# JJKK1313/DiTreeOnlinePlanner

Measured on AMD Instinct MI355X. Metric: candidate tree-expansions/sec (carmaze, H=32), higher is better.
Workload: dtype f16x3; 1 GPU; cfgs/carmaze.yaml + fm_policy flow sampler (K=1), batch=1024 candidates per GPU, H=32 (4 chunks x 8 steps), boxes.csv 20x20, 1024-node tree snapshot, seeded random weights; batch_per_gpu=1024, global_batch=1024, edge_length=32, action_horizon=8, pred_horizon=64, flow_steps=1, tree_nodes=1024, parallelism=candidates sharded x1

## Files before the change

### ditreeonlineplanner_amd/csrc/conv_tiles.hip

```cpp
#include <type_traits>

#include "denoise_device.h"

static thread_local bool g_dn_dry_run = false;
void denoise_set_dry_run(bool on) { g_dn_dry_run = on; }
bool denoise_dry_run() { return g_dn_dry_run; }

template <int PREC>
__device__ __forceinline__ void gemm_epilogue(const ConvGemmParams& p, f32x16_t (&acc)[2][4], char* smem, int tm, int tn,
                                              int tid, int lane, int r5, int h, int wm, int wn,
                                              long long out_extra_bytes = 0) {

  constexpr int ET = PREC == 2 ? 1 : 0;
  float satm = 0.0f;
  const int c_l = wn * 128 + 4 * r5;
  const int n0 = tn * 256 + c_l;
  const bool n_ok = n0 < p.N;
  float bias4[4] = {0.f, 0.f, 0.f, 0.f};
  if (p.bias != nullptr && n_ok) {
    f32x4_t t = *(const f32x4_t*)(p.bias + n0);
#pragma unroll
    for (int j = 0; j < 4; ++j) bias4[j] = t[j];
  }
#pragma unroll
// ... 352 lines not shown
#pragma unroll
      for (int i = 0; i < 16; ++i) acc[mb][j][i] = 0.0f;

  const int swl = (r5 >> 1) & 7;
  const int a_row_off = (wm * 64 + r5) * 128;
  const int b_row_off = 32768 + (wn * 128 + r5) * 128;

  auto kstep = [&](const char* sb, auto stage_tag, char* snext) {
    constexpr bool STAGE = decltype(stage_tag)::value;
    if constexpr (PREC != 1) {
      short8_t af[2][2], bfr[2][4];
      auto rd = [&](int ks, int slot) {
        const int ps = (((ks << 1) | h) ^ swl) << 4;
#pragma unroll
        for (int mb = 0; mb < 2; ++mb)
          af[slot][mb] = *(const short8_t*)(sb + a_row_off + mb * 4096 + ps);
#pragma unroll
        for (int j = 0; j < 4; ++j)
          bfr[slot][j] = *(const short8_t*)(sb + b_row_off + j * 4096 + ps);
      };
      if constexpr (STAGE) {
#pragma unroll
        for (int q = 0; q < 8; ++q) stage_piece(q, snext);
      }
      rd(0, 0);
#pragma unroll
      for (int ks = 0; ks < 4; ++ks) {
        if (ks < 3) rd(ks + 1, (ks + 1) & 1);
#pragma unroll
        for (int mb = 0; mb < 2; ++mb)
#pragma unroll
          for (int j = 0; j < 4; ++j)
            acc[mb][j] = mfma32<ET>(af[ks & 1][mb], bfr[ks & 1][j], acc[mb][j]);
      }
      if constexpr (STAGE) __builtin_amdgcn_sched_group_barrier(0x020, 8, 0);
      __builtin_amdgcn_sched_group_barrier(0x100, 6, 0);
#pragma unroll
      for (int ks = 0; ks < 4; ++ks) {
        if (ks < 3) __builtin_amdgcn_sched_group_barrier(0x100, 6, 0);
        __builtin_amdgcn_sched_group_barrier(0x008, 8, 0);
      }
    } else {
#pragma unroll
      for (int sl = 0; sl < 8; ++sl) {
        const int ps = (sl ^ swl) << 4;
        f32x4_t af[2], bfr[4];
#pragma unroll
        for (int mb = 0; mb < 2; ++mb) af[mb] = *(const f32x4_t*)(sb + a_row_off + mb * 4096 + ps);
#pragma unroll
        for (int j = 0; j < 4; ++j) bfr[j] = *(const f32x4_t*)(sb + b_row_off + j * 4096 + ps);
#pragma unroll
        for (int s2 = 0; s2 < 2; ++s2) {
#pragma unroll
          for (int mb = 0; mb < 2; ++mb) {
            const float a = h ? af[mb][2 * s2 + 1] : af[mb][2 * s2];
#pragma unroll
            for (int j = 0; j < 4; ++j) {
              const float bv = h ? bfr[j][2 * s2 + 1] : bfr[j][2 * s2];
              acc[mb][j] = __builtin_amdgcn_mfma_f32_32x32x2f32(a, bv, acc[mb][j], 0, 0, 0);
            }
          }
        }
        if constexpr (STAGE) stage_piece(sl, snext);
      }
    }
  };

#pragma unroll
  for (int q = 0; q < 8; ++q) stage_piece(q, smem);
  advance();
  for (int kt = 0; kt < nk - 1; ++kt) {
    asm volatile("s_waitcnt vmcnt(0)" ::: "memory");
    __syncthreads();
    kstep(smem + (kt & 1) * 65536, std::true_type{}, smem + ((kt + 1) & 1) * 65536);
    advance();
  }
  asm volatile("s_waitcnt vmcnt(0)" ::: "memory");
  __syncthreads();
  kstep(smem + ((nk - 1) & 1) * 65536, std::false_type{}, nullptr);
  __syncthreads();
  gemm_epilogue<PREC>(p, acc, smem, tm, tn, tid, lane, r5, h, wm, wn, out_extra);
}

template <int ET, bool SPLIT, bool SHORT = false>
__device__ __forceinline__ void gemm_epilogue16(const ConvGemmParams& p, f32x4_t (&acc)[4][8], char* smem, int tm, int tn,
                                                int tid, int lane, int r4, int h4, int wm, int wn) {
  const int c_l = wn * 128 + 8 * r4;
  const int n0 = tn * 256 + c_l;
  {
    f32x4_t b0 = {0.f, 0.f, 0.f, 0.f}, b1 = b0;
    if (p.bias != nullptr) { b0 = *(const f32x4_t*)(p.bias + n0); b1 = *(const f32x4_t*)(p.bias + n0 + 4); }
    if constexpr (ET == 1) {
      const float ws = p.w_scale;
#pragma unroll
      for (int mb = 0; mb < 4; ++mb)
#pragma unroll
        for (int j = 0; j < 4; ++j) { acc[mb][j] = acc[mb][j] * ws + b0[j]; acc[mb][4 + j] = acc[mb][4 + j] * ws + b1[j]; }
    } else if (p.bias != nullptr) {
#pragma unroll
      for (int mb = 0; mb < 4; ++mb)
#pragma unroll
        for (int j = 0; j < 4; ++j) { acc[mb][j] += b0[j]; acc[mb][4 + j] += b1[j]; }
    }
  }
  constexpr bool short_l = SHORT;
  const int lane_b = short_l ? (4 * h4) / p.L : 0, lane_l = -lane_b * p.L;
  int blk_b[4], blk_l[4];
#pragma unroll
  for (int mb = 0; mb < 4; ++mb) {
    const int m0 = tm * 256 + wm * 64 + mb * 16;
    const int b = m0 / p.L;
    blk_b[mb] = b;
    blk_l[mb] = m0 - b * p.L;
  }
  auto store_row = [&](char* o, const float (&v)[8]) {
    short8_t hi, lo;
    if constexpr (ET == 1) {
      sat_check_row(p.sat, v);
#pragma unroll
      for (int jj = 0; jj < 4; ++jj) {
        const f32x2_t c = {__builtin_amdgcn_fmed3f(v[2 * jj], -65504.0f, 65504.0f),
                           __builtin_amdgcn_fmed3f(v[2 * jj + 1], -65504.0f, 65504.0f)};
        const half2_t h = __builtin_convertvector(c, half2_t);
        const short2_t hs = __builtin_bit_cast(short2_t, h);
        hi[2 * jj] = hs[0]; hi[2 * jj + 1] = hs[1];
        if constexpr (SPLIT) {
          const half2_t l = __builtin_convertvector(c - __builtin_convertvector(h, f32x2_t), half2_t);
          const short2_t ls = __builtin_bit_cast(short2_t, l);
          lo[2 * jj] = ls[0]; lo[2 * jj + 1] = ls[1];
        }
      }
    } else {
#pragma unroll
      for (int j = 0; j < 8; ++j) {
        hi[j] = (short)f2bf(v[j]);
        if constexpr (SPLIT) lo[j] = (short)f2bf(v[j] - bf2f((unsigned short)hi[j]));
      }
    }
    *(short8_t*)o = hi;
    if constexpr (SPLIT) *(short8_t*)(o + p.out_plane) = lo;
  };
  auto out_ptr = [&](int mb, int esize) {
    const long long orow = (long long)(blk_b[mb] + lane_b) * p.out_Lp + (long long)(blk_l[mb] + 4 * h4 + lane_l) * p.out_stride + p.out_off;
    return (char*)p.Out + (orow * p.ldc + p.out_coff + n0) * esize;
  };
  if (p.mode < MODE_GN_MISH) {
    const int esize = p.out_f32 ? 4 : 2;
    const long long ostep = (long long)p.out_stride * p.ldc * esize;
#pragma unroll
    for (int mb = 0; mb < 4; ++mb) {
      char* ob = out_ptr(mb, esize);
#pragma unroll
      for (int i = 0; i < 4; ++i, ob += ostep) {
        float v[8];
#pragma unroll
        for (int j = 0; j < 8; ++j) v[j] = acc[mb][j][i];
        if (p.out_f32) {
          *(f32x4_t*)ob = f32x4_t{v[0], v[1], v[2], v[3]};
          *(f32x4_t*)(ob + 16) = f32x4_t{v[4], v[5], v[6], v[7]};
        } else {
          store_row(ob, v);
        }
      }
    }
    return;
  }
  const bool has_film = p.mode == MODE_GN_MISH_FILM, has_res = p.mode == MODE_GN_MISH_RES;
  const int spt = 256 / p.L;
  const int ns = spt > 16 ? spt * 4 : 64;
  float* s_sum = (float*)smem;
  float* s_sq = s_sum + ns;
  float* s_gb = s_sq + ns;
  float* s_film = s_gb + 512;
  const bool film_direct = has_film && short_l;
  const int b_last = p.M / p.L - 1;
  for (int i = tid; i < 2 * ns; i += 512) s_sum[i] = 0.0f;
  s_gb[tid] = tid < 256 ? p.gamma[tn * 256 + tid] : p.beta[tn * 256 + tid - 256];
  if (has_film && !film_direct) {
    for (int idx = tid; idx < spt * 128; idx += 512) {
      const int sm = idx >> 7, c4 = idx & 127;
      const int b = min(tm * spt + sm, b_last);
      const float* src = p.film + (long long)b * p.film_ld + p.film_off + tn * 256 + (c4 & 63) * 4 + (c4 >> 6) * p.N;
      *(f32x4_t*)(s_film + sm * 512 + c4 * 4) = *(const f32x4_t*)src;
    }
  }
  f32x4_t rh[2], rl[2];
  const long long rstep = (long long)p.ldres * 2;
  auto fetch_film = [&](int mb) {
    const float* fr = p.film + (long long)min(blk_b[mb] + lane_b, b_last) * p.film_ld + p.film_off + n0;
    rh[0] = *(const f32x4_t*)fr; rh[1] = *(const f32x4_t*)(fr + 4);
    rl[0] = *(const f32x4_t*)(fr + p.N); rl[1] = *(const f32x4_t*)(fr + p.N + 4);
  };
  if (film_direct) fetch_film(0);
  auto fetch_res = [&](int r) {
    const long long rrow = (long long)(blk_b[r >> 2] + lane_b) * p.res_Lp + blk_l[r >> 2] + 4 * h4 + lane_l + p.res_off;
    const char* rp = (const char*)p.Res + (rrow * p.ldres + n0) * 2 + (r & 3) * rstep;
    rh[r & 1] = *(const f32x4_t*)rp;
    if constexpr (SPLIT) rl[r & 1] = *(const f32x4_t*)(rp + p.res_plane);
  };
  if (has_res) { fetch_res(0); fetch_res(1); }
  __syncthreads();
  const int gi = c_l / p.group_ch;
  const bool wide = p.group_ch >= 128;
  const float inv_cnt = 1.0f / (float)(p.group_ch * p.L);
  int slot[4];
#pragma unroll
  for (int mb = 0; mb < 4; ++mb) slot[mb] = (blk_b[mb] + lane_b - tm * spt) * 4 + gi;
  const bool ordered = !short_l && (p.L >= 128 || (p.group_ch == 256 && p.L >= 32));
  const int hsame = short_l ? (p.L == 8 ? 2 : 1) : 4;
  const bool adder = (r4 == 0 || (!wide && r4 == 8)) && (h4 & (hsame - 1)) == 0;
  const int ocell = ((wm * 2 + wn) * 4 + gi) * 2;
  auto block_sums = [&](float (&s)[4], float* cell) {
#pragma unroll
    for (int mb = 0; mb < 4; ++mb) s[mb] = dpp_add<0xB1>(s[mb]);
#pragma unroll
    for (int mb = 0; mb < 4; ++mb) s[mb] = dpp_add<0x4E>(s[mb]);
#pragma unroll
    for (int mb = 0; mb < 4; ++mb) s[mb] = dpp_add<0x141>(s[mb]);
    if (wide) {
#pragma unroll
      for (int mb = 0; mb < 4; ++mb) s[mb] = dpp_add<0x140>(s[mb]);
    }
    if (hsame >= 2) {
#pragma unroll
      for (int mb = 0; mb < 4; ++mb) s[mb] += __shfl_xor(s[mb], 16);
    }
    if (hsame == 4) {
#pragma unroll
      for (int mb = 0; mb < 4; ++mb) s[mb] += __shfl_xor(s[mb], 32);
    }
    if (ordered) {
      if (p.L >= 64) { s[0] = (s[0] + s[1]) + (s[2] + s[3]); s[2] = 0.0f; }
      else { s[0] += s[1]; s[2] += s[3]; }
      if (adder) { cell[ocell] = s[0]; cell[ocell + 1] = s[2]; }
    } else if (adder) {
#pragma unroll
      for (int mb = 0; mb < 4; ++mb) atomicAdd(&cell[slot[mb]], s[mb]);
    }
  };
  auto cell_sums = [&](const float* cell, float (&t)[4]) {
    if (!ordered) {
#pragma unroll
      for (int mb = 0; mb < 4; ++mb) t[mb] = cell[slot[mb]];
      return;
    }
#pragma unroll
    for (int mb = 0; mb < 4; mb += 2) {
      const int r0 = (blk_b[mb] - tm * spt) * p.L;
      const int w0 = r0 >> 6, nw = p.L >= 64 ? p.L >> 6 : 1, sub = (r0 >> 5) & 1;
      float v = 0.0f;
      for (int w = w0; w < w0 + nw; ++w) {
        v += cell[((w * 2 + 0) * 4 + gi) * 2 + sub];
        v += cell[((w * 2 + 1) * 4 + gi) * 2 + sub];
      }
      t[mb] = v; t[mb + 1] = v;
    }
  };
  float mean_[4], rstd_[4];
  auto pair = [&](int mb, int j, int ip) { return f32x2_t{acc[mb][j][2 * ip], acc[mb][j][2 * ip + 1]}; };
  if constexpr (!SPLIT) {
    float s[4], q[4];
#pragma unroll
    for (int mb = 0; mb < 4; ++mb) {
      f32x2_t s2 = {0.f, 0.f}, q2 = {0.f, 0.f};
#pragma unroll
      for (int j = 0; j < 8; ++j)
#pragma unroll
        for (int ip = 0; ip < 2; ++ip) {
          const f32x2_t v = pair(mb, j, ip);
          s2 += v;
          q2 = __builtin_elementwise_fma(v, v, q2);
        }
      s[mb] = s2[0] + s2[1];
      q[mb] = q2[0] + q2[1];
    }
    block_sums(s, s_sum);
    block_sums(q, s_sq);
    __syncthreads();
    cell_sums(s_sum, s);
    cell_sums(s_sq, q);
#pragma unroll
    for (int mb = 0; mb < 4; ++mb) {
      mean_[mb] = s[mb] * inv_cnt;
      const float var = fmaxf(q[mb] * inv_cnt - mean_[mb] * mean_[mb], 0.0f);
// ... 108 lines not shown
template <int ET>
__device__ __forceinline__ void mm16_snake(f32x4_t (&acc)[4][8], const short8_t (&a)[4], const short8_t (&b)[4], int half) {
#pragma unroll
  for (int mb = 0; mb < 4; ++mb)
#pragma unroll
    for (int jj = 0; jj < 4; ++jj) {
      const int j = (mb & 1) ? 3 - jj : jj;
      acc[mb][half * 4 + j] = mfma16<ET>(a[mb], b[j], acc[mb][half * 4 + j]);
    }
}

#ifdef HALO16_STAMP
__device__ unsigned long long g_halo_stamp[8];
extern "C" int ditree_debug_halo_stamp(unsigned long long* out) {
  return (int)hipMemcpyFromSymbol(out, HIP_SYMBOL(g_halo_stamp), sizeof(g_halo_stamp));
}
__device__ unsigned int g_x3_phase[8][32];
extern "C" int ditree_debug_x3_phase(unsigned int* out) {
  return (int)hipMemcpyFromSymbol(out, HIP_SYMBOL(g_x3_phase), sizeof(g_x3_phase));
}
#define X3_STAMP_MAX 65536
__device__ unsigned long long g_x3_stamp[X3_STAMP_MAX][6];
__device__ unsigned int g_x3_count;
extern "C" int ditree_debug_x3_stamp(unsigned long long* out, unsigned int* count, int reset) {
  int rc = (int)hipMemcpyFromSymbol(count, HIP_SYMBOL(g_x3_count), 4);
  if (rc == 0 && out != nullptr) rc = (int)hipMemcpyFromSymbol(out, HIP_SYMBOL(g_x3_stamp), sizeof(unsigned long long) * 6 * X3_STAMP_MAX);
  if (rc == 0 && reset) { unsigned int z = 0; rc = (int)hipMemcpyToSymbol(HIP_SYMBOL(g_x3_count), &z, 4); }
  return rc;
}
#endif
template <int ET>
__global__ void __launch_bounds__(512, 2) conv3_halo16_kernel(ConvGemmParams p) {
  extern __shared__ __attribute__((aligned(16))) char smem[];
  constexpr int A_BUF = 40960, W_BUF = 32768, W_BASE = 2 * A_BUF;
  const int tid = threadIdx.x, lane = tid & 63;
  const int w = __builtin_amdgcn_readfirstlane(tid >> 6);
  const int r4 = lane & 15, h4 = lane >> 4;
  const int wm = w >> 1, wn = w & 1;
  const int ntn = (p.N + 255) >> 8;
  const int ntm = (p.M + 255) >> 8;
  const int tile = xcd_remap_strips(blockIdx.x, ntm, ntn, p.xcd_strips);
  const int tm = tile / ntn, tn = tile - tm * ntn;
  const int L = p.L, Lp = p.in_Lp, S = 256 / L;
  const int a_rows = S * Lp;
  const int nc = p.Cin >> 6;
  const long long K = 3LL * p.Cin;

  unsigned pa0, pa4, pb;
  const char* const a_base = (const char*)p.A + ((long long)tm * S * Lp + p.in_off) * p.lda * 2;
  const char* const w_base = (const char*)p.W + ((long long)tn * 256) * K * 2;
  const __amdgpu_buffer_rsrc_t a_rsrc = __builtin_amdgcn_make_buffer_rsrc((void*)a_base, 0, 0x7fffffff, 0x00020000);
  const __amdgpu_buffer_rsrc_t w_rsrc = __builtin_amdgcn_make_buffer_rsrc((void*)w_base, 0, 0x7fffffff, 0x00020000);
  {
    const int r = w * 8 + (lane >> 3);
    const int slot = (lane & 7) ^ (r & 7);
    pa0 = (unsigned)((r * p.lda + slot * 8) * 2);
    const int r4r = r + 256;
    const int rs = r4r < a_rows ? r4r : a_rows - 1;
    pa4 = (unsigned)((rs * p.lda + slot * 8) * 2);
  }
  const int a_piece = 64 * p.lda * 2;
  long long wq[4];
  {
    const int lr = lane >> 3;
    const int slot = (lane & 7) ^ lr;
    pb = (unsigned)(((long long)(8 * lr) * K + slot * 8) * 2);
#pragma unroll
    for (int q = 0; q < 4; ++q) {
      const int r0 = (w * 4 + q) * 8;
      const int cu = (r0 & 128) + 8 * (r0 & 8) + ((r0 >> 4) & 7);
      wq[q] = (long long)cu * K * 2;
    }
  }
  const int w_tap = p.Cin * 2;
  auto issue_a = [&](int c, int i) {
    __builtin_amdgcn_raw_ptr_buffer_load_lds(a_rsrc, (LDS_AS void*)(smem + (c & 1) * A_BUF + (w + 8 * i) * 1024), 16,
                                             i < 4 ? pa0 : pa4, c * 128 + (i < 4 ? i * a_piece : 0), 0, 0);
  };
  auto issue_w = [&](int c, int t, int q) {
    __builtin_amdgcn_raw_ptr_buffer_load_lds(w_rsrc, (LDS_AS void*)(smem + W_BASE + ((c + t) & 1) * W_BUF + (w * 4 + q) * 1024),
                                             16, pb, (int)wq[q] + c * 128 + t * w_tap, 0, 0);
  };

  int lrow0;
  {
    const int ml = wm * 64 + r4;
    const int sb = ml / L;
    lrow0 = sb * Lp + (ml - sb * L);
  }
  int lstep[4];
#pragma unroll
  for (int mb = 0; mb < 4; ++mb) lstep[mb] = 16 * mb + 2 * (((wm * 64 + 16 * mb) / L) - ((wm * 64) / L));
  const int swl = r4 & 7;
  const int b_row_off = (wn * 128 + r4) * 128;

  f32x4_t acc[4][8];
#pragma unroll
  for (int mb = 0; mb < 4; ++mb)
#pragma unroll
    for (int j = 0; j < 8; ++j) acc[mb][j] = f32x4_t{0.f, 0.f, 0.f, 0.f};

  short8_t af[2][4], bq[2][4];
  auto rdA = [&](int set, int c, int t, int ks) {
    const char* ab = smem + (c & 1) * A_BUF;
#pragma unroll
    for (int mb = 0; mb < 4; ++mb) {
      const int row = lrow0 + lstep[mb] + t;
      const int ps = (((ks << 2) | h4) ^ (row & 7)) << 4;
      af[set][mb] = *(const short8_t*)(ab + row * 128 + ps);
    }
  };
  auto rdB = [&](int set, int c, int t, int ks, int half) {
    const char* wb = smem + W_BASE + ((c + t) & 1) * W_BUF + b_row_off + half * 8192;
    const int psb = (((ks << 2) | h4) ^ swl) << 4;
#pragma unroll
    for (int jj = 0; jj < 4; ++jj) bq[set][jj] = *(const short8_t*)(wb + jj * 2048 + psb);
  };
  auto mm = [&](int aset, int bset, int half, int mb, int jj) {
    acc[mb][half * 4 + jj] = mfma16<ET>(af[aset][mb], bq[bset][jj], acc[mb][half * 4 + jj]);
  };
  auto mm16 = [&](int aset, int bset, int half) { mm16_snake<ET>(acc, af[aset], bq[bset], half); };

  auto step = [&](auto tT, auto tNext, auto tIW, auto tIA, auto tVM, int c) {
    constexpr int T = decltype(tT)::value;
    constexpr bool HAS_NEXT = decltype(tNext)::value, ISSUE_W = decltype(tIW)::value, ISSUE_A = decltype(tIA)::value;
    constexpr int VM = decltype(tVM)::value;
    constexpr int NV = ISSUE_W ? 4 : 0;
    asm volatile("" : "+v"(lrow0));
    __builtin_amdgcn_s_setprio(2);
    rdB(1, c, T, 0, 1);
    mm16(0, 0, 0);
    __builtin_amdgcn_sched_group_barrier(0x100, 4, 0);
    __builtin_amdgcn_sched_group_barrier(0x008, 16, 0);
    __builtin_amdgcn_sched_barrier(0);
    __builtin_amdgcn_s_setprio(1);
    rdA(1, c, T, 1);
    rdB(0, c, T, 1, 0);
    mm16(0, 1, 1);
    __builtin_amdgcn_sched_group_barrier(0x100, 8, 0);
    __builtin_amdgcn_sched_group_barrier(0x008, 16, 0);
    __builtin_amdgcn_sched_barrier(0);
    __builtin_amdgcn_s_setprio(0);
    rdB(1, c, T, 1, 1);
    mm16(1, 0, 0);
    if constexpr (ISSUE_A && T != 2) {
      if constexpr (T == 0) { issue_a(c + 1, 0); issue_a(c + 1, 1); issue_a(c + 1, 2); }
      else { issue_a(c + 1, 3); issue_a(c + 1, 4); }
      __builtin_amdgcn_sched_group_barrier(0x100, 4, 0);
      __builtin_amdgcn_sched_group_barrier(0x008, 4, 0);
      __builtin_amdgcn_sched_group_barrier(0x020, 1, 0);
      __builtin_amdgcn_sched_group_barrier(0x008, 4, 0);
      __builtin_amdgcn_sched_group_barrier(0x020, 1, 0);
      __builtin_amdgcn_sched_group_barrier(0x008, 4, 0);
      if constexpr (T == 0) __builtin_amdgcn_sched_group_barrier(0x020, 1, 0);
      __builtin_amdgcn_sched_group_barrier(0x008, 4, 0);
    } else {
      __builtin_amdgcn_sched_group_barrier(0x100, 4, 0);
      __builtin_amdgcn_sched_group_barrier(0x008, 16, 0);
    }
    __builtin_amdgcn_sched_barrier(0);
    if constexpr (HAS_NEXT) {
      if constexpr (VM == 0) asm volatile("s_waitcnt vmcnt(0) lgkmcnt(0)" ::: "memory");
      else if constexpr (VM == 3) asm volatile("s_waitcnt vmcnt(3) lgkmcnt(0)" ::: "memory");
      else asm volatile("s_waitcnt vmcnt(2) lgkmcnt(0)" ::: "memory");
      __builtin_amdgcn_s_barrier();
      __builtin_amdgcn_s_setprio(3);
      constexpr int T1 = (T + 1) % 3;
      rdA(0, c + (T + 1) / 3, T1, 0);
      rdB(0, c + (T + 1) / 3, T1, 0, 0);
    }
    constexpr int T2 = (T + 2) % 3;
    const int c2 = c + (T + 2) / 3;
#pragma unroll
    for (int mb = 0; mb < 4; ++mb)
#pragma unroll
      for (int jj = 0; jj < 4; ++jj) {
        mm(1, 1, 1, mb, (mb & 1) ? 3 - jj : jj);
        const int i = mb * 4 + jj;
        const int d = (i & 1) ? -1 : (i >> 1);
        if constexpr (ISSUE_W) { if (d >= 0 && d < 4) issue_w(c2, T2, d); }
      }
    if constexpr (HAS_NEXT) __builtin_amdgcn_sched_group_barrier(0x100, 8, 1);
#pragma unroll
    for (int i = 0; i < 16; ++i) {
      __builtin_amdgcn_sched_group_barrier(0x008, 1, 1);
      if (!(i & 1) && (i >> 1) < NV) __builtin_amdgcn_sched_group_barrier(0x020, 1, 1);
    }
    __builtin_amdgcn_sched_barrier(0);
  };
  using I0 = std::integral_constant<int, 0>;
  using I1 = std::integral_constant<int, 1>;
  using I2 = std::integral_constant<int, 2>;
  using I3 = std::integral_constant<int, 3>;
  using Tt = std::true_type;
  using Ff = std::false_type;

#pragma unroll
  for (int i = 0; i < 5; ++i) issue_a(0, i);
#pragma unroll
  for (int q = 0; q < 4; ++q) issue_w(0, 0, q);
  asm volatile("s_waitcnt vmcnt(0)" ::: "memory");
  __builtin_amdgcn_s_barrier();
#pragma unroll
  for (int q = 0; q < 4; ++q) issue_w(0, 1, q);
  rdA(0, 0, 0, 0);
  rdB(0, 0, 0, 0, 0);

#ifdef HALO16_STAMP
  const unsigned long long st0 = __builtin_amdgcn_s_memtime(), rt0 = __builtin_amdgcn_s_memrealtime();
#endif
  for (int c = 0; c < nc - 2; ++c) {
    step(I0{}, Tt{}, Tt{}, Tt{}, I3{}, c);
    step(I1{}, Tt{}, Tt{}, Tt{}, I2{}, c);
    step(I2{}, Tt{}, Tt{}, Tt{}, I0{}, c);
  }
#ifdef HALO16_STAMP
  if (blockIdx.x == 100 && tid == 0 && nc >= 32) {
    g_halo_stamp[0] = __builtin_amdgcn_s_memtime() - st0;
    g_halo_stamp[1] = __builtin_amdgcn_s_memrealtime() - rt0;
    g_halo_stamp[2] = (unsigned long long)(nc - 2) * 3;
  }
#endif
  {
    const int c = nc - 2;
    step(I0{}, Tt{}, Tt{}, Tt{}, I0{}, c);
    step(I1{}, Tt{}, Tt{}, Tt{}, I0{}, c);
    step(I2{}, Tt{}, Tt{}, Ff{}, I0{}, c);
  }
  {
    const int c = nc - 1;
    step(I0{}, Tt{}, Tt{}, Ff{}, I0{}, c);
    step(I1{}, Tt{}, Ff{}, Ff{}, I0{}, c);
    step(I2{}, Ff{}, Ff{}, Ff{}, I0{}, c);
  }
  __builtin_amdgcn_s_setprio(0);
  __syncthreads();
  gemm_epilogue16<ET, false>(p, acc, smem, tm, tn, tid, lane, r4, h4, wm, wn);
}

template <int ET, bool SHORT = false, bool SPLITK = false, int NP = 5>
__global__ void __launch_bounds__(512, 2) conv3_halo16x3_kernel(ConvGemmParams p) {
  extern __shared__ __attribute__((aligned(16))) char smem[];
  static_assert(NP == 5 || NP == 6, "five or six activation pieces");
  constexpr int A_BUF = NP * 8192, W_BUF = 32768, W_BASE = 2 * A_BUF;
  const int tid = threadIdx.x, lane = tid & 63;
  const int w = __builtin_amdgcn_readfirstlane(tid >> 6);
  const int r4 = lane & 15, h4 = lane >> 4;
  const int wm = w >> 1, wn = w & 1;
  const int ntn = (p.N + 255) >> 8;
  const int ntm = (p.M + 255) >> 8;
  const int tile = xcd_remap_strips(blockIdx.x, ntm, ntn, p.xcd_strips);
  const int tm = tile / ntn, tn = tile - tm * ntn;
  const int L = p.L, Lp = p.in_Lp, S = 256 / L;
  const int a_rows = S * Lp;
  const int nv_all = p.Cin >> 5;
  const int v_lo = SPLITK ? (int)blockIdx.y * (nv_all / p.splitk) : 0;
  const int nv = SPLITK ? v_lo + nv_all / p.splitk : nv_all;
  const long long K = 3LL * p.Cin;
  const unsigned a_plane = (unsigned)p.a_plane, w_plane = (unsigned)p.w_plane;

  unsigned pa0, pa4, pa5 = 0, pb;
  const char* const a_base = (const char*)p.A + ((long long)tm * S * Lp + p.in_off) * p.lda * 2;
  const char* const w_base = (const char*)p.W + ((long long)tn * 256) * K * 2;
  const __amdgpu_buffer_rsrc_t a_rsrc = __builtin_amdgcn_make_buffer_rsrc((void*)a_base, 0, 0x7fffffff, 0x00020000);
  const __amdgpu_buffer_rsrc_t w_rsrc = __builtin_amdgcn_make_buffer_rsrc((void*)w_base, 0, 0x7fffffff, 0x00020000);
  {
    const int r = w * 8 + (lane >> 3);
    const int slot = (lane & 7) ^ (r & 7);
    const unsigned po = (slot & 4) ? a_plane : 0u;
    pa0 = (unsigned)((r * p.lda + (slot & 3) * 8) * 2) + po;
    const int r4r = r + 256;
    const int rs = r4r < a_rows ? r4r : a_rows - 1;
    pa4 = (unsigned)((rs * p.lda + (slot & 3) * 8) * 2) + po;
    if constexpr (NP == 6) {
      const int r5r = r + 320;
      const int rs5 = r5r < a_rows ? r5r : a_rows - 1;
      pa5 = (unsigned)((rs5 * p.lda + (slot & 3) * 8) * 2) + po;
    }
  }
  const int a_piece = 64 * p.lda * 2;
  long long wq[4];
  {
    const int lr = lane >> 3;
    const int slot = (lane & 7) ^ lr;
    pb = (unsigned)(((long long)(8 * lr) * K + (slot & 3) * 8) * 2) + ((slot & 4) ? w_plane : 0u);
#pragma unroll
    for (int q = 0; q < 4; ++q) {
      const int r0 = (w * 4 + q) * 8;
      const int cu = (r0 & 128) + 8 * (r0 & 8) + ((r0 >> 4) & 7);
      wq[q] = (long long)cu * K * 2;
    }
  }
  const int w_tap = p.Cin * 2;
  auto issue_a = [&](int v, int i) {
    __builtin_amdgcn_raw_ptr_buffer_load_lds(a_rsrc, (LDS_AS void*)(smem + (v & 1) * A_BUF + (w + 8 * i) * 1024), 16,
                                             i < 4 ? pa0 : (i == 4 ? pa4 : pa5), v * 64 + (i < 4 ? i * a_piece : 0), 0, 0);
  };
  auto issue_w = [&](int v, int t, int q) {
    __builtin_amdgcn_raw_ptr_buffer_load_lds(w_rsrc, (LDS_AS void*)(smem + W_BASE + ((v + t) & 1) * W_BUF + (w * 4 + q) * 1024),
                                             16, pb, (int)wq[q] + v * 64 + t * w_tap, 0, 0);
  };

  int lrow0;
  {
    const int ml = wm * 64 + r4;
    const int sb = ml / L;
    lrow0 = sb * Lp + (ml - sb * L);
  }
  int lstep[4];
#pragma unroll
  for (int mb = 0; mb < 4; ++mb) lstep[mb] = 16 * mb + 2 * (((wm * 64 + 16 * mb) / L) - ((wm * 64) / L));
  const int swl = r4 & 7;
  const int b_row_off = (wn * 128 + r4) * 128;

  f32x4_t acc[4][8];
#pragma unroll
  for (int mb = 0; mb < 4; ++mb)
#pragma unroll
    for (int j = 0; j < 8; ++j) acc[mb][j] = f32x4_t{0.f, 0.f, 0.f, 0.f};

  short8_t af[2][4], bq[2][4];
  auto rdA = [&](int set, int v, int t, int pl) {
    const char* ab = smem + (v & 1) * A_BUF;
#pragma unroll
    for (int mb = 0; mb < 4; ++mb) {
      const int row = lrow0 + lstep[mb] + t;
      const int ps = (((pl << 2) | h4) ^ (row & 7)) << 4;
      af[set][mb] = *(const short8_t*)(ab + row * 128 + ps);
    }
  };
  auto rdB = [&](int set, int v, int t, int pl, int half) {
    const char* wb = smem + W_BASE + ((v + t) & 1) * W_BUF + b_row_off + half * 8192;
    const int psb = (((pl << 2) | h4) ^ swl) << 4;
#pragma unroll
    for (int jj = 0; jj < 4; ++jj) bq[set][jj] = *(const short8_t*)(wb + jj * 2048 + psb);
  };
  auto mm = [&](int aset, int bset, int half, int mb, int jj) {
    acc[mb][half * 4 + jj] = mfma16<ET>(af[aset][mb], bq[bset][jj], acc[mb][half * 4 + jj]);
  };
  auto mm16 = [&](int aset, int bset, int half) { mm16_snake<ET>(acc, af[aset], bq[bset], half); };

#ifdef X3_PHASE_STAMP
  unsigned pst[24];
#define PSTAMP(k) do { pst[T * 8 + (k)] = (unsigned)__builtin_amdgcn_s_memtime(); __builtin_amdgcn_sched_barrier(0); } while (0)
#else
#define PSTAMP(k) do { } while (0)
#endif
  auto step = [&](auto tT, auto tNext, auto tIW, auto tIA, auto tVM, int v) {
    constexpr int T = decltype(tT)::value;
    constexpr bool HAS_NEXT = decltype(tNext)::value, ISSUE_W = decltype(tIW)::value, ISSUE_A = decltype(tIA)::value;
    constexpr int VM = decltype(tVM)::value;
    asm volatile("" : "+v"(lrow0));
    PSTAMP(0);
    __builtin_amdgcn_s_setprio(2);
    rdB(1, v, T, 1, 1);
    mm16(0, 0, 0);
    __builtin_amdgcn_sched_group_barrier(0x100, 4, 0);
    __builtin_amdgcn_sched_group_barrier(0x008, 16, 0);
    __builtin_amdgcn_sched_barrier(0);
    PSTAMP(1);
    rdB(0, v, T, 0, 0);
    rdA(1, v, T, 1);
    mm16(0, 1, 1);
    __builtin_amdgcn_sched_group_barrier(0x100, 8, 0);
    __builtin_amdgcn_sched_group_barrier(0x008, 16, 0);
    __builtin_amdgcn_sched_barrier(0);
    PSTAMP(2);
    __builtin_amdgcn_s_setprio(1);
    rdB(1, v, T, 0, 1);
    mm16(0, 0, 0);
    __builtin_amdgcn_sched_group_barrier(0x100, 4, 0);
    __builtin_amdgcn_sched_group_barrier(0x008, 16, 0);
    __builtin_amdgcn_sched_barrier(0);
    PSTAMP(3);
    mm16(1, 0, 0);
    if constexpr (ISSUE_A && T != 2) {
      if constexpr (T == 0) { issue_a(v + 1, 0); issue_a(v + 1, 1); issue_a(v + 1, 2); }
      else { issue_a(v + 1, 3); issue_a(v + 1, 4); if constexpr (NP == 6) issue_a(v + 1, 5); }
      __builtin_amdgcn_sched_group_barrier(0x008, 4, 2);
      __builtin_amdgcn_sched_group_barrier(0x020, 1, 2);
      __builtin_amdgcn_sched_group_barrier(0x008, 4, 2);
      __builtin_amdgcn_sched_group_barrier(0x020, 1, 2);
      __builtin_amdgcn_sched_group_barrier(0x008, 4, 2);
      if constexpr (T == 0 || NP == 6) __builtin_amdgcn_sched_group_barrier(0x020, 1, 2);
      __builtin_amdgcn_sched_group_barrier(0x008, 4, 2);
    }
    __builtin_amdgcn_sched_barrier(0);
    PSTAMP(4);
    __builtin_amdgcn_s_setprio(0);
    mm16(0, 1, 1);
    __builtin_amdgcn_sched_barrier(0);
    PSTAMP(5);
    if constexpr (HAS_NEXT) {
      if constexpr (VM == 0) asm volatile("s_waitcnt vmcnt(0) lgkmcnt(0)" ::: "memory");
      else if constexpr (VM == 3) asm volatile("s_waitcnt vmcnt(3) lgkmcnt(0)" ::: "memory");
      else asm volatile("s_waitcnt vmcnt(2) lgkmcnt(0)" ::: "memory");
      __builtin_amdgcn_s_barrier();
      __builtin_amdgcn_s_setprio(3);
      PSTAMP(6);
      constexpr int T1 = (T + 1) % 3;
      rdA(0, v + (T + 1) / 3, T1, 0);
      rdB(0, v + (T + 1) / 3, T1, 1, 0);
    }
    constexpr int T2 = (T + 2) % 3;
    const int v2 = v + (T + 2) / 3;
#pragma unroll
    for (int mb = 0; mb < 4; ++mb)
#pragma unroll
      for (int jj = 0; jj < 4; ++jj) {
        mm(1, 1, 1, mb, (mb & 1) ? 3 - jj : jj);
        const int i = mb * 4 + jj;
        const int d = (i & 1) ? -1 : (i >> 1);
        if constexpr (ISSUE_W) { if (d >= 0 && d < 4) issue_w(v2, T2, d); }
      }
    if constexpr (HAS_NEXT) __builtin_amdgcn_sched_group_barrier(0x100, 8, 1);
    constexpr int NV = ISSUE_W ? 4 : 0;
#pragma unroll
    for (int i = 0; i < 16; ++i) {
      __builtin_amdgcn_sched_group_barrier(0x008, 1, 1);
      if (!(i & 1) && (i >> 1) < NV) __builtin_amdgcn_sched_group_barrier(0x020, 1, 1);
    }
    __builtin_amdgcn_sched_barrier(0);
    PSTAMP(7);
  };
#undef PSTAMP
  using I0 = std::integral_constant<int, 0>;
  using I1 = std::integral_constant<int, 1>;
  using I2 = std::integral_constant<int, 2>;
  using I3 = std::integral_constant<int, 3>;
  using Tt = std::true_type;
  using Ff = std::false_type;

#ifdef HALO16_STAMP
  const unsigned long long xs0 = __builtin_amdgcn_s_memrealtime();
#endif
#pragma unroll
  for (int i = 0; i < NP; ++i) issue_a(v_lo, i);
#pragma unroll
  for (int q = 0; q < 4; ++q) issue_w(v_lo, 0, q);
  asm volatile("s_waitcnt vmcnt(0)" ::: "memory");
  __builtin_amdgcn_s_barrier();
#pragma unroll
  for (int q = 0; q < 4; ++q) issue_w(v_lo, 1, q);
  rdA(0, v_lo, 0, 0);
  rdB(0, v_lo, 0, 1, 0);
#ifdef HALO16_STAMP
  const unsigned long long xs1 = __builtin_amdgcn_s_memrealtime();
#endif

  using IT1 = std::integral_constant<int, NP == 6 ? 3 : 2>;
  for (int v = v_lo; v < nv - 2; ++v) {
    step(I0{}, Tt{}, Tt{}, Tt{}, I3{}, v);
    step(I1{}, Tt{}, Tt{}, Tt{}, IT1{}, v);
    step(I2{}, Tt{}, Tt{}, Tt{}, I0{}, v);
  }
#ifdef X3_PHASE_STAMP
  if (blockIdx.x == 100 && lane == 0 && nv == 64) {
#pragma unroll
    for (int k = 0; k < 24; ++k) g_x3_phase[w][k] = pst[k];
    g_x3_phase[w][24] = (unsigned)nv;
  }
#endif
  {
    const int v = nv - 2;
    step(I0{}, Tt{}, Tt{}, Tt{}, I0{}, v);
    step(I1{}, Tt{}, Tt{}, Tt{}, I0{}, v);
    step(I2{}, Tt{}, Tt{}, Ff{}, I0{}, v);
  }
  {
    const int v = nv - 1;
    step(I0{}, Tt{}, Tt{}, Ff{}, I0{}, v);
    step(I1{}, Tt{}, Ff{}, Ff{}, I0{}, v);
    step(I2{}, Ff{}, Ff{}, Ff{}, I0{}, v);
  }
  __builtin_amdgcn_s_setprio(0);
  __syncthreads();
#ifdef HALO16_STAMP
  const unsigned long long xs2 = __builtin_amdgcn_s_memrealtime();
#endif
  if constexpr (SPLITK) {
    const int ntiles = ntm * ntn;
    float* mine = p.sk_ws + ((size_t)blockIdx.y * ntiles + tile) * 65536;
#pragma unroll
    for (int mb = 0; mb < 4; ++mb)
#pragma unroll
      for (int j = 0; j < 8; ++j) *(f32x4_t*)(mine + ((mb * 8 + j) * 512 + tid) * 4) = acc[mb][j];
    __threadfence();
    __syncthreads();
    int* s_last = (int*)smem;
    if (tid == 0) *s_last = atomicAdd(p.sk_cnt + tile, 1) == p.splitk - 1;
    __syncthreads();
    const bool last = *s_last != 0;
    __syncthreads();
    if (!last) return;
    __threadfence();
#pragma unroll
    for (int mb = 0; mb < 4; ++mb)
#pragma unroll
      for (int j = 0; j < 8; ++j) acc[mb][j] = f32x4_t{0.f, 0.f, 0.f, 0.f};
    for (int sp = 0; sp < p.splitk; ++sp) {
      const float* sl = p.sk_ws + ((size_t)sp * ntiles + tile) * 65536;
#pragma unroll
      for (int mb = 0; mb < 4; ++mb)
#pragma unroll
        for (int j = 0; j < 8; ++j) acc[mb][j] += *(const f32x4_t*)(sl + ((mb * 8 + j) * 512 + tid) * 4);
    }
    if (tid == 0) p.sk_cnt[tile] = 0;
  }
  gemm_epilogue16<ET, true, SHORT>(p, acc, smem, tm, tn, tid, lane, r4, h4, wm, wn);
#ifdef HALO16_STAMP
  __syncthreads();
  if (tid == 0) {
    const unsigned long long xs3 = __builtin_amdgcn_s_memrealtime();
    const unsigned int k = atomicAdd(&g_x3_count, 1u);
    if (k < X3_STAMP_MAX) {
      g_x3_stamp[k][0] = xs0; g_x3_stamp[k][1] = xs1; g_x3_stamp[k][2] = xs2; g_x3_stamp[k][3] = xs3;
      g_x3_stamp[k][4] = ((unsigned long long)nv << 32) | blockIdx.x;
      g_x3_stamp[k][5] = ((unsigned long long)__builtin_amdgcn_s_getreg((31 << 11) | 20) << 32) |
                         (unsigned int)__builtin_amdgcn_s_getreg((31 << 11) | 4);
    }
  }
#endif
}

template <int ET, bool SPLIT>
__global__ void __launch_bounds__(256) conv2d_small_kernel(ConvGemmParams p) {
  extern __shared__ __attribute__((aligned(16))) char smem[];
  constexpr int STAGE = 16384;
  constexpr int CK = SPLIT ? 32 : 64;
  const int tid = threadIdx.x, lane = tid & 63;
  const int w = __builtin_amdgcn_readfirstlane(tid >> 6);
  const int r5 = lane & 31, h = lane >> 5;
  const int wm = w >> 1, wn = w & 1;
  const int ntn = p.N >> 6;
  const int tm = blockIdx.x / ntn, tn = blockIdx.x - tm * ntn;
  const int kpt = p.Cin / CK;
  const long long K = (long long)p.taps * p.Cin;
  int k0 = 0, nk = p.taps * kpt;
  long long out_extra = 0;
  if (p.splitk > 1) {
    const int per = (nk + p.splitk - 1) / p.splitk;
    k0 = blockIdx.y * per;
    nk = min(nk - k0, per);
    out_extra = (long long)blockIdx.y * p.slab_stride;
  }

  const char* a_base[2];
  int ih0[2], iw0[2];
  const char* w_src[2];
  int slot_b[2];
  long long plane_a[2];
#pragma unroll
  for (int q = 0; q < 2; ++q) {
    const int r = (2 * w + q) * 8 + (lane >> 3);
    const int slot = (lane & 7) ^ ((r >> 1) & 7);
    slot_b[q] = SPLIT ? (slot & 3) * 16 : slot * 16;
    plane_a[q] = (SPLIT && (slot & 4)) ? p.a_plane : 0;
    const long long plane_w = (SPLIT && (slot & 4)) ? p.w_plane : 0;
    int m = tm * 64 + r;
    m = m < p.M ? m : p.M - 1;
    const int b = m / p.c2_OHW, rem = m - b * p.c2_OHW;
    const int oh = rem / p.c2_OW, ow = rem - oh * p.c2_OW;
    a_base[q] = (const char*)p.A + (long long)b * p.c2_H * p.c2_W * p.Cin * 2;
    ih0[q] = oh * p.c2_stride - p.c2_pad;
    iw0[q] = ow * p.c2_stride - p.c2_pad;
    w_src[q] = (const char*)p.W + ((long long)(tn * 64 + r) * K) * 2 + slot_b[q] + plane_w;
  }
  auto issue = [&](int kl) {
    const int k = k0 + kl;
    const int tap = k / kpt, kin = k - tap * kpt;
    const int kh = p.c2_kh[tap], kw = p.c2_kw[tap];
    char* st = smem + (kl % 3) * STAGE;
#pragma unroll
    for (int q = 0; q < 2; ++q) {
      const int ih = ih0[q] + kh, iw = iw0[q] + kw;
      const bool ok = ih >= 0 && ih < p.c2_H && iw >= 0 && iw < p.c2_W;
      const char* src = ok ? a_base[q] + ((long long)(ih * p.c2_W + iw) * p.Cin + kin * CK) * 2 + plane_a[q] : (const char*)p.zero;
      __builtin_amdgcn_global_load_lds((const GLOBAL_AS void*)(src + slot_b[q]), (LDS_AS void*)(st + (2 * w + q) * 1024), 16, 0, 0);
    }
#pragma unroll
    for (int q = 0; q < 2; ++q)
      __builtin_amdgcn_global_load_lds((const GLOBAL_AS void*)(w_src[q] + (long long)k * (CK * 2)),
                                       (LDS_AS void*)(st + 8192 + (2 * w + q) * 1024), 16, 0, 0);
  };

  f32x16_t acc;
#pragma unroll
  for (int i = 0; i < 16; ++i) acc[i] = 0.0f;
  const int a_row = wm * 32 + r5, b_row = wn * 32 + r5;
  const int a_off = a_row * 128, b_off = 8192 + b_row * 128;
  const int sa = (a_row >> 1) & 7, sb = (b_row >> 1) & 7;

// ... 376 lines not shown
```

Measured before the change: 19280 candidate expansions/s.

## Prefetch epilogue gamma/beta/FiLM into LDS during final conv mainloop phases

Adds an epilogue request plan whose gamma, beta and FiLM rows are issued as buffer-to-LDS loads inside the last two MFMA phases of the halo conv kernels, interleaved with the remaining matrix math. The epilogue then skips its own global loads and one barrier, and a single vmcnt wait before the final sync covers the prefetched data. This is meant to hide the epilogue parameter fetch latency behind compute, at the cost of more scalar registers for the plan and tighter LDS buffer reuse (writing into the free A buffer). The split-K variant keeps the old path.

```diff
diff --git a/ditreeonlineplanner_amd/csrc/conv_tiles.hip b/ditreeonlineplanner_amd/csrc/conv_tiles.hip
--- a/ditreeonlineplanner_amd/csrc/conv_tiles.hip
+++ b/ditreeonlineplanner_amd/csrc/conv_tiles.hip
@@ -458,7 +458,43 @@
   gemm_epilogue<PREC>(p, acc, smem, tm, tn, tid, lane, r5, h, wm, wn, out_extra);
 }
 
-template <int ET, bool SPLIT, bool SHORT = false>
+constexpr int EPI_REQ = 5;
+struct EpiPlan {
+  unsigned long long src[EPI_REQ];
+  int dst[EPI_REQ];
+  int records[EPI_REQ];
+};
+template <bool SHORT>
+__device__ __forceinline__ void epi_plan(EpiPlan& e, const ConvGemmParams& p, int tm, int tn, int w, int spt, int b_last) {
+  const int ne = p.mode < MODE_GN_MISH ? 0 : ((p.mode == MODE_GN_MISH_FILM && !SHORT) ? 2 + 2 * spt : 2);
+  const int ns = spt > 16 ? spt * 4 : 64;
+  const unsigned long long ga = (unsigned long long)(p.gamma + tn * 256), be = (unsigned long long)(p.beta + tn * 256);
+#pragma unroll
+  for (int k = 0; k < EPI_REQ; ++k) {
+    const int idx = min(w + 8 * k, ne);
+    int rec = w + 8 * k < ne ? 1024 : 0;
+    const int b = min(tm * spt + ((idx - 2) >> 1), b_last);
+    unsigned long long fi =
+        (unsigned long long)p.film + (unsigned long long)(((long long)b * p.film_ld + p.film_off + tn * 256 + (idx & 1) * p.N) * 4);
+    asm volatile("" : "+s"(fi));
+    unsigned long long a = idx == 0 ? ga : (idx == 1 ? be : fi);
+    int d = 2 * ns * 4 + idx * 1024;
+    asm volatile("" : "+s"(a), "+s"(d), "+s"(rec));
+    e.src[k] = a;
+    e.dst[k] = d;
+    e.records[k] = rec;
+  }
+}
+__device__ __forceinline__ void epi_request(const EpiPlan& e, char* img, int k, unsigned lane16) {
+  const __amdgpu_buffer_rsrc_t rsrc = __builtin_amdgcn_make_buffer_rsrc((void*)e.src[k], 0, e.records[k], 0x00020000);
+  __builtin_amdgcn_raw_ptr_buffer_load_lds(rsrc, (LDS_AS void*)(img + e.dst[k]), 16, lane16, 0, 0, 0);
+}
+__device__ __forceinline__ void epi_zero_cells(char* img, int tid, int spt) {
+  const int ns = spt > 16 ? spt * 4 : 64;
+  ((float*)img)[min(tid, 2 * ns - 1)] = 0.0f;
+}
+
+template <int ET, bool SPLIT, bool SHORT = false, bool PRE = false>
 __device__ __forceinline__ void gemm_epilogue16(const ConvGemmParams& p, f32x4_t (&acc)[4][8], char* smem, int tm, int tn,
                                                 int tid, int lane, int r4, int h4, int wm, int wn) {
   const int c_l = wn * 128 + 8 * r4;
@@ -550,14 +586,16 @@
   float* s_film = s_gb + 512;
   const bool film_direct = has_film && short_l;
   const int b_last = p.M / p.L - 1;
-  for (int i = tid; i < 2 * ns; i += 512) s_sum[i] = 0.0f;
-  s_gb[tid] = tid < 256 ? p.gamma[tn * 256 + tid] : p.beta[tn * 256 + tid - 256];
-  if (has_film && !film_direct) {
-    for (int idx = tid; idx < spt * 128; idx += 512) {
-      const int sm = idx >> 7, c4 = idx & 127;
-      const int b = min(tm * spt + sm, b_last);
-      const float* src = p.film + (long long)b * p.film_ld + p.film_off + tn * 256 + (c4 & 63) * 4 + (c4 >> 6) * p.N;
-      *(f32x4_t*)(s_film + sm * 512 + c4 * 4) = *(const f32x4_t*)src;
+  if constexpr (!PRE) {
+    for (int i = tid; i < 2 * ns; i += 512) s_sum[i] = 0.0f;
+    s_gb[tid] = tid < 256 ? p.gamma[tn * 256 + tid] : p.beta[tn * 256 + tid - 256];
+    if (has_film && !film_direct) {
+      for (int idx = tid; idx < spt * 128; idx += 512) {
+        const int sm = idx >> 7, c4 = idx & 127;
+        const int b = min(tm * spt + sm, b_last);
+        const float* src = p.film + (long long)b * p.film_ld + p.film_off + tn * 256 + (c4 & 63) * 4 + (c4 >> 6) * p.N;
+        *(f32x4_t*)(s_film + sm * 512 + c4 * 4) = *(const f32x4_t*)src;
+      }
     }
   }
   f32x4_t rh[2], rl[2];
@@ -575,7 +613,7 @@
     if constexpr (SPLIT) rl[r & 1] = *(const f32x4_t*)(rp + p.res_plane);
   };
   if (has_res) { fetch_res(0); fetch_res(1); }
-  __syncthreads();
+  if constexpr (!PRE) __syncthreads();
   const int gi = c_l / p.group_ch;
   const bool wide = p.group_ch >= 128;
   const float inv_cnt = 1.0f / (float)(p.group_ch * p.L);
@@ -850,6 +888,10 @@
                                              16, pb, (int)wq[q] + c * 128 + t * w_tap, 0, 0);
   };
 
+  char* const e_img = smem + (nc & 1) * A_BUF;
+  EpiPlan eplan;
+  auto issue_e = [&](int k) { epi_request(eplan, e_img, k, (unsigned)lane * 16u); };
+
   int lrow0;
   {
     const int ml = wm * 64 + r4;
@@ -889,11 +931,12 @@
   };
   auto mm16 = [&](int aset, int bset, int half) { mm16_snake<ET>(acc, af[aset], bq[bset], half); };
 
-  auto step = [&](auto tT, auto tNext, auto tIW, auto tIA, auto tVM, int c) {
+  auto step_ep = [&](auto tT, auto tNext, auto tIW, auto tIA, auto tVM, auto tEP, int c) {
     constexpr int T = decltype(tT)::value;
     constexpr bool HAS_NEXT = decltype(tNext)::value, ISSUE_W = decltype(tIW)::value, ISSUE_A = decltype(tIA)::value;
-    constexpr int VM = decltype(tVM)::value;
-    constexpr int NV = ISSUE_W ? 4 : 0;
+    constexpr int VM = decltype(tVM)::value, EP = decltype(tEP)::value;
+    static_assert(!(ISSUE_W && EP != 0), "one kind of request per phase");
+    constexpr int NV = (ISSUE_W || EP == 1) ? 4 : (EP == 2 ? 1 : 0);
     asm volatile("" : "+v"(lrow0));
     __builtin_amdgcn_s_setprio(2);
     rdB(1, c, T, 0, 1);
@@ -947,6 +990,8 @@
         const int i = mb * 4 + jj;
         const int d = (i & 1) ? -1 : (i >> 1);
         if constexpr (ISSUE_W) { if (d >= 0 && d < 4) issue_w(c2, T2, d); }
+        if constexpr (EP == 1) { if (d >= 0 && d < 4) issue_e(d); }
+        if constexpr (EP == 2) { if (d == 0) issue_e(4); }
       }
     if constexpr (HAS_NEXT) __builtin_amdgcn_sched_group_barrier(0x100, 8, 1);
 #pragma unroll
@@ -962,6 +1007,7 @@
   using I3 = std::integral_constant<int, 3>;
   using Tt = std::true_type;
   using Ff = std::false_type;
+  auto step = [&](auto tT, auto tNext, auto tIW, auto tIA, auto tVM, int c) { step_ep(tT, tNext, tIW, tIA, tVM, I0{}, c); };
 
 #pragma unroll
   for (int i = 0; i < 5; ++i) issue_a(0, i);
@@ -989,6 +1035,7 @@
     g_halo_stamp[2] = (unsigned long long)(nc - 2) * 3;
   }
 #endif
+  epi_plan<false>(eplan, p, tm, tn, w, S, ntm * S - 1);
   {
     const int c = nc - 2;
     step(I0{}, Tt{}, Tt{}, Tt{}, I0{}, c);
@@ -998,12 +1045,14 @@
   {
     const int c = nc - 1;
     step(I0{}, Tt{}, Tt{}, Ff{}, I0{}, c);
-    step(I1{}, Tt{}, Ff{}, Ff{}, I0{}, c);
-    step(I2{}, Ff{}, Ff{}, Ff{}, I0{}, c);
+    step_ep(I1{}, Tt{}, Ff{}, Ff{}, I0{}, I1{}, c);
+    step_ep(I2{}, Ff{}, Ff{}, Ff{}, I0{}, I2{}, c);
   }
   __builtin_amdgcn_s_setprio(0);
+  epi_zero_cells(e_img, tid, S);
+  asm volatile("s_waitcnt vmcnt(0)" ::: "memory");
   __syncthreads();
-  gemm_epilogue16<ET, false>(p, acc, smem, tm, tn, tid, lane, r4, h4, wm, wn);
+  gemm_epilogue16<ET, false, false, true>(p, acc, e_img, tm, tn, tid, lane, r4, h4, wm, wn);
 }
 
 template <int ET, bool SHORT = false, bool SPLITK = false, int NP = 5>
@@ -1069,6 +1118,10 @@
                                              16, pb, (int)wq[q] + v * 64 + t * w_tap, 0, 0);
   };
 
+  constexpr bool PRE = !SPLITK;
+  EpiPlan eplan;
+  auto issue_e = [&](int k) { epi_request(eplan, smem, k, (unsigned)lane * 16u); };
+
   int lrow0;
   {
     const int ml = wm * 64 + r4;
@@ -1114,10 +1167,11 @@
 #else
 #define PSTAMP(k) do { } while (0)
 #endif
-  auto step = [&](auto tT, auto tNext, auto tIW, auto tIA, auto tVM, int v) {
+  auto step_ep = [&](auto tT, auto tNext, auto tIW, auto tIA, auto tVM, auto tEP, int v) {
     constexpr int T = decltype(tT)::value;
     constexpr bool HAS_NEXT = decltype(tNext)::value, ISSUE_W = decltype(tIW)::value, ISSUE_A = decltype(tIA)::value;
-    constexpr int VM = decltype(tVM)::value;
+    constexpr int VM = decltype(tVM)::value, EP = decltype(tEP)::value;
+    static_assert(!(ISSUE_W && EP != 0), "one kind of request per P6");
     asm volatile("" : "+v"(lrow0));
     PSTAMP(0);
     __builtin_amdgcn_s_setprio(2);
@@ -1180,9 +1234,11 @@
         const int i = mb * 4 + jj;
         const int d = (i & 1) ? -1 : (i >> 1);
         if constexpr (ISSUE_W) { if (d >= 0 && d < 4) issue_w(v2, T2, d); }
+        if constexpr (EP == 1) { if (d >= 0 && d < 4) issue_e(d); }
+        if constexpr (EP == 2) { if (d == 0) issue_e(4); }
       }
     if constexpr (HAS_NEXT) __builtin_amdgcn_sched_group_barrier(0x100, 8, 1);
-    constexpr int NV = ISSUE_W ? 4 : 0;
+    constexpr int NV = (ISSUE_W || EP == 1) ? 4 : (EP == 2 ? 1 : 0);
 #pragma unroll
     for (int i = 0; i < 16; ++i) {
       __builtin_amdgcn_sched_group_barrier(0x008, 1, 1);
@@ -1198,6 +1254,7 @@
   using I3 = std::integral_constant<int, 3>;
   using Tt = std::true_type;
   using Ff = std::false_type;
+  auto step = [&](auto tT, auto tNext, auto tIW, auto tIA, auto tVM, int v) { step_ep(tT, tNext, tIW, tIA, tVM, I0{}, v); };
 
 #ifdef HALO16_STAMP
   const unsigned long long xs0 = __builtin_amdgcn_s_memrealtime();
@@ -1229,6 +1286,7 @@
     g_x3_phase[w][24] = (unsigned)nv;
   }
 #endif
+  if constexpr (PRE) epi_plan<SHORT>(eplan, p, tm, tn, w, S, ntm * S - 1);
   {
     const int v = nv - 2;
     step(I0{}, Tt{}, Tt{}, Tt{}, I0{}, v);
@@ -1238,10 +1296,14 @@
   {
     const int v = nv - 1;
     step(I0{}, Tt{}, Tt{}, Ff{}, I0{}, v);
-    step(I1{}, Tt{}, Ff{}, Ff{}, I0{}, v);
-    step(I2{}, Ff{}, Ff{}, Ff{}, I0{}, v);
+    step_ep(I1{}, Tt{}, Ff{}, Ff{}, I0{}, std::integral_constant<int, PRE ? 1 : 0>{}, v);
+    step_ep(I2{}, Ff{}, Ff{}, Ff{}, I0{}, std::integral_constant<int, PRE ? 2 : 0>{}, v);
   }
   __builtin_amdgcn_s_setprio(0);
+  if constexpr (PRE) {
+    epi_zero_cells(smem, tid, S);
+    asm volatile("s_waitcnt vmcnt(0)" ::: "memory");
+  }
   __syncthreads();
 #ifdef HALO16_STAMP
   const unsigned long long xs2 = __builtin_amdgcn_s_memrealtime();
@@ -1275,7 +1337,7 @@
     }
     if (tid == 0) p.sk_cnt[tile] = 0;
   }
-  gemm_epilogue16<ET, true, SHORT>(p, acc, smem, tm, tn, tid, lane, r4, h4, wm, wn);
+  gemm_epilogue16<ET, true, SHORT, PRE>(p, acc, smem, tm, tn, tid, lane, r4, h4, wm, wn);
 #ifdef HALO16_STAMP
   __syncthreads();
   if (tid == 0) {
```

Result: no change. 19320 candidate expansions/s, median of 2 (+0.2%).
